# elador/FeatureDetection

Measured on AMD Instinct MI355X. Metric: Mpatches/s (extract+WVM+SVM) per GPU, 640x480 pyramid, higher is better.
Workload: dtype u8/i32/f32/f64; 1 GPU; config 1/metric config: ffpDetectApp FaceFrontal.cfg five-stage cascade on 640x480 BGR frames: 13-layer pyramid, 20x20 windows step 1 (16185 windows/frame), HistEq64 -> WVM 280 filters -> OE -> RBF-SVM 1024 SV -> NMS; fd_pyramid_update_frames + fd_detect_five_stage_frames (the frames of a call share one pyramid aren...; frames_per_call=64, calls_in_flight=11, parallelism=image-shard dp1

## Files before the change

### featuredetection_amd/capi.py

```python
import ctypes as C
import os
import numpy as np

_HERE = os.path.dirname(os.path.abspath(__file__))
LIB_PATH = os.environ.get("FD_HIP_LIB", os.path.join(_HERE, "libfd_hip.so"))

FD_OK, FD_ERR_INVALID_ARGUMENT, FD_ERR_RUNTIME, FD_ERR_LOGIC, FD_ERR_HIP, FD_ERR_CAPACITY, FD_ERR_DEVICE_CAPACITY = range(7)
FD_LAYER_NONE, FD_LAYER_GRADBIN, FD_LAYER_LBP = 0, 1, 2
IMAGE_GRAY, IMAGE_GREYWORLD_GRAY = 0, 1
FD_KERNEL_LINEAR, FD_KERNEL_POLY, FD_KERNEL_RBF, FD_KERNEL_HIK = 0, 1, 2, 3
FD_DTYPE_U8, FD_DTYPE_F32 = 0, 1


class FdError(RuntimeError):
    def __init__(self, code, msg):
        super().__init__("fd_hip error %d: %s" % (code, msg))
        self.code = code


class fd_wvm_model(C.Structure):
    _fields_ = [("filter_w", C.c_int32), ("filter_h", C.c_int32), ("num_filters", C.c_int32), ("num_used", C.c_int32),
                ("num_per_level", C.c_int32), ("basis_param", C.c_float), ("bias", C.c_float),
                ("thresholds", C.POINTER(C.c_float)), ("hk_weights", C.POINTER(C.c_float)), ("pp", C.POINTER(C.c_double)),
                ("val_off", C.POINTER(C.c_int32)), ("val", C.POINTER(C.c_double)), ("rec_off", C.POINTER(C.c_int32)),
# ... 326 lines not shown
    "fd_gradient_sum_length": (C.c_int, [C.c_int, C.c_int, C.c_int, C.c_int]),
    "fd_surf_feature_length": (C.c_int, [C.c_int, C.c_int]),
}

_BENCH_SIGS = {
    "fd_debug_svm_u8_both": (C.c_int, [C.c_void_p, C.c_void_p, C.c_void_p, C.c_int64, C.c_void_p, C.c_void_p]),
    "fd_ctx_set_kernel_timing": (C.c_int, [C.c_void_p, C.c_int]),
    "fd_last_kernel_ms": (C.c_int, [C.c_void_p, C.POINTER(C.c_char_p), C.POINTER(C.c_float)]),
    "fd_last_group_prefilter_ms": (C.c_int, [C.c_void_p, C.POINTER(C.c_float), C.POINTER(C.c_int)]),
    "fd_debug_wvb_rect_sums": (C.c_int64, [C.POINTER(fd_wvm_model), C.c_void_p, C.c_int64, C.c_void_p, C.c_void_p]),
    "fd_wvm_last_queue_length": (C.c_int64, [C.c_void_p]),
    "fd_wvm_last_tail_state": (C.c_int, [C.c_void_p]),
    "fd_wvm_last_spec_state": (C.c_int, [C.c_void_p]),
    "fd_wvm_last_stage_b_plan": (C.c_int, [C.c_void_p, C.c_void_p]),
    "fd_debug_wvd_plan": (C.c_int, [C.c_void_p, C.c_void_p, C.c_int, C.c_int, C.c_int, C.c_int, C.c_int, C.c_void_p]),
}


def lib():
    global _lib
    if _lib is None:
        if not os.path.exists(LIB_PATH):
            raise ImportError("%s not built: run `python -c 'import __graft_entry__ as g; g.build()'` "
                              "(hipcc --offload-arch=gfx950); there is no CPU fallback" % LIB_PATH)
        l = C.CDLL(LIB_PATH)
        for name, (res, args) in list(_SIGS.items()) + list(_BENCH_SIGS.items()):
            f = getattr(l, name)
            f.restype = res
            f.argtypes = args
        _lib = l
# ... 286 lines not shown

def svm_u8_both(ctx, svm, feats):
    feats = _c(feats, np.uint8).reshape(-1, svm.dim)
    o8, o16 = np.empty(len(feats), np.float64), np.empty(len(feats), np.float64)
    ctx.check(lib().fd_debug_svm_u8_both(ctx.h, svm.h, _ptr(feats), len(feats), _ptr(o8), _ptr(o16)))
    return o8, o16


def wvd_plan(nx, ny, frames, sy, ph, slots):
    nx, ny = _c(nx, np.int32), _c(ny, np.int32)
    first = np.zeros(len(nx) + 1, np.int32)
    k = lib().fd_debug_wvd_plan(_ptr(nx), _ptr(ny), len(nx), frames, sy, ph, slots, _ptr(first))
    if k < 1:
        raise FdError(k, "fd_debug_wvd_plan")
    return k, first


def wvb_rect_sums(model, patches_eq):
    s, keep = _wvm_struct(model, fd_wvm_model)
    patches_eq = _c(patches_eq, np.uint8)
    n = patches_eq.shape[0]
    gen = np.zeros(5, np.int32)
    ncols = lib().fd_debug_wvb_rect_sums(C.byref(s), None, 0, None, _ptr(gen))
    if ncols < 0:
        return None
    out = np.empty((n, ncols), np.int32)
    lib().fd_debug_wvb_rect_sums(C.byref(s), _ptr(patches_eq), n, _ptr(out), None)
    return out, [int(g) for g in gen if g >= 0]


# ... 1211 lines not shown
```

### featuredetection_amd/csrc/fd_internal.hpp

```cpp
#pragma once
#include <hip/hip_runtime.h>
#include <chrono>
#include <cstdint>
#include <cstdio>
#include <cstdlib>
#include <cmath>
#include <map>
#include <memory>
#include <string>
#include <typeindex>
#include <typeinfo>
#include <vector>
#include <stdexcept>
#include <atomic>
#include <condition_variable>
#include <functional>
#include <mutex>
#include <thread>
#include <deque>
#include <exception>
#include "../../include/fd_hip.h"
#include "../../include/fd_hip_bench.h"

struct FdPinned {
// ... 249 lines not shown
    }
    return ctx->tail;
}

static inline int fd_env_int(const char* name, int dflt, int lo, int hi) {
    const char* e = getenv(name);
    const int v = e ? atoi(e) : dflt;
    return v < lo ? lo : (v > hi ? hi : v);
}
static inline int fd_knob_batch_threads() { static const int v = fd_env_int("FD_BATCH_THREADS", 8, 1, 16); return v; }
static inline int fd_knob_wvd_rounds() { static const int v = fd_env_int("FD_WVD_ROUNDS", 2, 1, 64); return v; }
static inline bool fd_knob_trace() { static const bool on = getenv("FD_TRACE") != nullptr; return on; }
static inline int fd_knob_fs_tail() { const char* e = getenv("FD_FS_TAIL"); return e ? atoi(e) : -1; }
static inline bool fd_knob_fs_spec() { const char* e = getenv("FD_FS_SPEC"); return !(e && atoi(e) == 0); }
static inline bool fd_knob_cond_device() { const char* e = getenv("FD_COND_DEVICE"); return e && atoi(e) == 1; }

struct FdStopwatch {
    bool on = fd_knob_trace();
    std::chrono::steady_clock::time_point t;
    FdStopwatch() { restart(); }
    void restart() { if (on) t = std::chrono::steady_clock::now(); }
    int64_t lap_ns() {
        if (!on) return 0;
        const std::chrono::steady_clock::time_point n = std::chrono::steady_clock::now();
        const int64_t ns = std::chrono::duration_cast<std::chrono::nanoseconds>(n - t).count();
        t = n;
        return ns;
    }
};

// ... 127 lines not shown
```

### featuredetection_amd/csrc/pyramid.hip

```cpp
#include "fd_internal.hpp"
#include "fd_device.hpp"
#include <algorithm>
#include <cstring>

namespace {

constexpr int MAXJ = 16;

struct ResizeJob {
    int dw, dh;
    uint32_t dst_off;
    double scale_x, scale_y;
};
struct ResizeJobs {
    int n;
    ResizeJob j[MAXJ];
};
struct DownJob {
    int sw, sh;
    uint32_t src_off, dst_off;
};
struct FusedJob {
    int dw0, dh0, dw1, dh1;
    uint32_t dst0_off;
// ... 349 lines not shown
    }
#ifdef FD_PYR_PROF
    if (threadIdx.x == 0 && blockIdx.x < (unsigned int)PYR_PROF_WGS) {
        for (int i = 0; i < 6; ++i) fd_pyr_prof[blockIdx.x * 8 + i] = pacc[i];
        fd_pyr_prof[blockIdx.x * 8 + 6] = ptiles;
    }
#endif
}

__device__ __forceinline__ int reflect_cf(int p, int len) {
    int q = p < 0 ? -p : p;
    q = q >= len ? 2 * len - 2 - q : q;
    return min(max(q, 0), len - 1);
}
constexpr int PD_W = 62;
__global__ __launch_bounds__(256) void k_pyrdown_tiled(uint8_t* __restrict__ arena, DownJobs jobs, size_t imageStride) {
    __shared__ __attribute__((aligned(16))) uint8_t tile[TL_ROWS * TL_PITCH];
    arena += (size_t)blockIdx.z * imageStride;
    const int c = threadIdx.x & 63, rq = __builtin_amdgcn_readfirstlane(threadIdx.x >> 6);
    constexpr int NROWS = 2 * PD_TH + 3, PD_LD = (NROWS + 7) / 8;
    static_assert(2 * (3 + 4 * (PD_LD - 1)) + 1 < TL_ROWS && 128 <= TL_PITCH && 2 * PD_W + 3 <= 128, "pyrDown stage");
    for (int g = blockIdx.x; g < jobs.tile0[jobs.n]; g += gridDim.x) {
        int ji = 0;
        while (ji + 1 < jobs.n && g >= jobs.tile0[ji + 1]) ++ji;
        const DownJob jb = jobs.j[ji];
        const int t = g - jobs.tile0[ji];
        const int sw = jb.sw, sh = jb.sh;
        const int dw = (sw + 1) / 2, dh = (sh + 1) / 2;
        const uint8_t* src = arena + jb.src_off;
        uint8_t* dst = arena + jb.dst_off;
        const int tilesX = (dw + PD_W - 1) / PD_W;
        const int ty = t / tilesX, tx = t - ty * tilesX;
        const int dx0 = tx * PD_W, dy0 = ty * PD_TH;
        const int X0 = 2 * dx0 - 2, Y0 = 2 * dy0 - 2;
        {
            const int j4 = 4 * (c & 31), half = c >> 5;
            const int xs = X0 + j4;
// ... 633 lines not shown
        const int gx = std::max(1, std::min((int)((npix / 4 + 1023) / 1024), perFrame));
        hipLaunchKernelGGL(k_gw_stats, dim3(gx, NI), dim3(256), 0, st, fp, stats, (int)npix);
        hipLaunchKernelGGL(k_gw_gray, dim3(gx, NI), dim3(256), 0, st, fp, stats, gray, IS, (int)npix);
    } else if (frames) {
        hipLaunchKernelGGL(k_frames_to_gray, dim3(grid_for((int)(npix / 16 + 1)), NI), dim3(256), 0, st, fp, gray, IS, (int)npix, ch);
    } else if (ch == 3) {
        hipLaunchKernelGGL(k_bgr2gray, dim3(grid_for((int)npix)), dim3(256), 0, st, fp.p[0], gray, (int)npix);
    } else {
        HIP_CHECK(hipMemcpyAsync(gray, fp.p[0], npix, hipMemcpyDeviceToDevice, st));
    }
    const fd_pyramid::Plan& plan = *p->plan;
    for (const ResizeLaunch& R : plan.resize)
        hipLaunchKernelGGL(k_resize_tiled, dim3(R.grid, R.jobs.n, NI), dim3(256), 0, st, arena, arena, p->gray_full_off, W, H, R.jobs, IS);
    for (const FusedLaunch& F : plan.fused)
        hipLaunchKernelGGL(k_resize_down, dim3(F.grid), dim3(256), 0, st, arena, p->gray_full_off, W, H, p->rtab.as<int2>(), F.jobs, F.tileTab, F.tilesPerFrame, NI, IS);
    for (const DownLaunch& D : plan.down)
        hipLaunchKernelGGL(k_pyrdown_tiled, dim3(tile_grid_for(D.jobs.tile0[D.jobs.n]), 1, NI), dim3(256), 0, st, arena, D.jobs, IS);
    for (const FilterLaunch& F : plan.filter) {
        const dim3 g(F.grid, F.jobs.n);
        if (F.blur.n) hipLaunchKernelGGL(k_box_blur, g, dim3(256), 0, st, arena, p->grad_blur, F.blur);
        if (p->filter_kind != FD_LAYER_GRADBIN)
            hipLaunchKernelGGL(k_lbp, g, dim3(256), 0, st, arena, p->lbp_type, F.jobs);
        else if (p->interpolate)
            hipLaunchKernelGGL(k_gradbin<4>, g, dim3(256), 0, st, arena, p->lut.as<uint8_t>(), p->grad_kernel, F.jobs);
        else
            hipLaunchKernelGGL(k_gradbin<2>, g, dim3(256), 0, st, arena, p->lut.as<uint8_t>(), p->grad_kernel, F.jobs);
    }
    HIP_CHECK(hipGetLastError());
    if (!p->ready) HIP_CHECK(hipEventCreateWithFlags(&p->ready, hipEventDisableTiming));
    HIP_CHECK(hipEventRecord(p->ready, st));
    p->readyStream = st;
    p->version++;
// ... 383 lines not shown
```

### featuredetection_amd/csrc/wvm.hip

```cpp
#include "fd_internal.hpp"
#include "five_stage_stages.hpp"
#include <chrono>
#include <thread>
#include <algorithm>
#include <cstring>
#include <memory>
#include <mutex>
#include <atomic>


struct fd_svm;
int fd_svm_dim(const fd_svm* m);
bool fd_svm_is_u8(const fd_svm* m);
float fd_svm_threshold(const fd_svm* m);
double fd_svm_probability(const fd_svm* m, double d);
void fd_svm_generic_launch(fd_ctx* ctx, const fd_svm* m, const void* dfeat, const uint32_t* didx, int64_t stride_bytes, int64_t n, double* dout);
void fd_svm_generic_launch_on(hipStream_t st, const fd_svm* m, const void* dfeat, const uint32_t* didx, int64_t stride_bytes, int64_t n, double* dout);
bool fd_svm_u8_mfma_available(const fd_svm* m);
void fd_svm_u8_mfma_launch_counted(hipStream_t st, const fd_svm* m, const void* dfeat, const uint32_t* didx, int64_t stride_bytes, int64_t nmax,
                                   const unsigned int* dcount, double* dout);

constexpr int WVM_MAX_LAYERS = 64;
constexpr int WVM_MAX_DIM = 32;
constexpr int WVM_MAX_VALS = 16;
// ... 1146 lines not shown
        m->sbAux[i].reserve(sizeof(int2) * (size_t)cap);
        m->sbU[i].reserve(sizeof(float) * (size_t)mv.numPer * 64 * tilesCap);
        m->sbK[i].reserve(sizeof(float) * (size_t)mv.numUsed * 64 * tilesCap);
        s.X[i] = m->sbX[i].as<int8_t>(); s.wid[i] = m->sbWid[i].as<int64_t>(); s.aux[i] = m->sbAux[i].as<int2>();
        s.U[i] = m->sbU[i].as<float>(); s.K[i] = m->sbK[i].as<float>();
    }
    m->sbKey.reserve(sizeof(unsigned long long) * (size_t)cap);
    s.exitKey = m->sbKey.as<unsigned long long>();
    s.cnt = m->sbCnt.as<unsigned int>();
    s.cap = cap;
    m->deepCap = cap;
}

static int wvd_plan_sliding(WvdTable& t, int K) {
    t.K = K;
    int tiles = 0;
    for (int i = 0; i < t.n; ++i) {
        WvdLayer& l = t.l[i];
        l.G = (l.ny + K - 1) / K;
        l.sTileFirst = tiles;
        tiles += (int)(((int64_t)l.nx * l.G + 63) / 64);
    }
    t.sTilesPerImage = tiles;
    return tiles;
}
static int wvd_choose_k(WvdTable t, int slots, int ph) {
    static const int forced = [] { const char* e = getenv("FD_WVD_K"); const int v = e ? atoi(e) : 0; return v < 1 ? 0 : (v > WVD_KMAX ? WVD_KMAX : v); }();
    if (2 * t.sy > ph) return 1;
    if (forced) return forced;
    int best = 1;
    double bestCost = 0;
    for (int K = 1; K <= WVD_KMAX; ++K) {
        const int64_t tiles = (int64_t)wvd_plan_sliding(t, K) * t.nimg;
        const double rounds = (double)((tiles + slots - 1) / slots);
        const double cost = rounds * (0.45 + K * (1.0 + (K > 1 ? 0.04 * t.sy : 0.0)));
        if (K == 1 || cost < bestCost * 0.999) { best = K; bestCost = cost; }
    }
    return best;
}

template <int PW_, int PH_>
static void launch_prefilter_sized(fd_ctx* ctx, hipStream_t st, const uint8_t* arena, WvdTable wt, const WvdDev& dv) {
    static int perCu = 0;
    if (perCu == 0 && (hipOccupancyMaxActiveBlocksPerMultiprocessor(&perCu, k_wvm_prefilter<PW_, PH_>, 256, 0) != hipSuccess || perCu < 1)) perCu = 2;
    const int slots = ctx->num_cus * perCu * 4;
    const int64_t tiles = (int64_t)wvd_plan_sliding(wt, wvd_choose_k(wt, slots, PH_)) * wt.nimg;
    int grid = (int)std::min<int64_t>((tiles + 3) / 4, (int64_t)ctx->num_cus * perCu * fd_knob_wvd_rounds());
    if (wt.nimg >= 8 && grid >= 64) grid &= ~7;
    hipLaunchKernelGGL((k_wvm_prefilter<PW_, PH_>), dim3(grid), dim3(256), 0, st, arena, wt, dv);
}

static bool wvd_table_from(const WinTable& wt, WvdTable& t) {
    if (wt.raw || wt.list || wt.total < 512) return false;
    std::memset(&t, 0, sizeof(t));
    t.n = wt.n; t.sx = wt.sx; t.sy = wt.sy;
    const int64_t perImage = wt.nimg > 1 ? wt.per_image : wt.total;
    int tiles = 0;
    for (int i = 0; i < wt.n; ++i) {
        const WinLayerDev& s = wt.l[i];
        const int64_t nwin = (i + 1 < wt.n ? wt.l[i + 1].first : perImage) - s.first;
        if (nwin <= 0 || nwin > (int64_t)INT32_MAX - 64) return false;
// ... 15 lines not shown
    dv.c = m->denseC.as<WvdConst>();
    dv.q = q;
    dv.qcount = qcount;
    dv.L = m->denseL;
    dv.negBasis = m->dev.negBasis; dv.negBias = m->dev.negBias; dv.stretch = m->dev.stretch;
    dv.sxxSlack = (float)(2 * m->dev.fh + 2);
    dv.scale = m->denseScale;
    dv.nb2 = (double)m->dev.negBasis * 1.4426950408889634;
    dv.mXq = -2.0 * m->denseScale * dv.nb2;
}

static bool launch_prefilter(fd_ctx* ctx, hipStream_t st, fd_wvm* m, const uint8_t* arena, const WinTable& wt, int64_t* q, unsigned int* qcount) {
    if (m->denseL == 0) return false;
    WvdTable t;
    if (!wvd_table_from(wt, t)) return false;
    WvdDev dv;
    wvd_dev_from(m, q, qcount, dv);
#define FD_WVM_CASE(W, H) \
    if (m->dev.fw == W && m->dev.fh == H) { launch_prefilter_sized<W, H>(ctx, st, arena, t, dv); return true; }
    FD_WVM_CASE(20, 20) FD_WVM_CASE(24, 24) FD_WVM_CASE(16, 24) FD_WVM_CASE(32, 16) FD_WVM_CASE(32, 24)
#undef FD_WVM_CASE
    return false;
}

template <int PW_, int PH_>
static void launch_prefilter_group_sized(fd_ctx* ctx, hipStream_t st, const uint8_t* arena, WvdTable wt, const WvdGroup& g) {
    static int perCu = 0;
    if (perCu == 0 && (hipOccupancyMaxActiveBlocksPerMultiprocessor(&perCu, k_wvm_prefilter_group<PW_, PH_>, 256, 0) != hipSuccess || perCu < 1)) perCu = 2;
    const int slots = ctx->num_cus * perCu * 4;
    const int64_t tiles = (int64_t)wvd_plan_sliding(wt, wvd_choose_k(wt, slots, PH_)) * wt.nimg;
// ... 719 lines not shown
    std::memset(&t, 0, sizeof(t));
    t.n = n_layers; t.sx = 1; t.sy = sy; t.nimg = frames;
    for (int i = 0; i < n_layers; ++i) {
        if (nx[i] < 1 || ny[i] < 1) return FD_ERR_INVALID_ARGUMENT;
        t.l[i].nx = nx[i]; t.l[i].ny = ny[i];
    }
    const int K = wvd_choose_k(t, slots, ph);
    const int tiles = wvd_plan_sliding(t, K);
    if (tile_first) {
        for (int i = 0; i < n_layers; ++i) tile_first[i] = t.l[i].sTileFirst;
        tile_first[n_layers] = tiles;
    }
    return K;
}

int64_t fd_debug_wvb_rect_sums(const fd_wvm_model* md, const uint8_t* patches, int64_t n, int32_t* out, int32_t* phase_gen ) {
    if (!md || md->num_filters < 1) return -1;
    const int NU = (md->num_used > md->num_filters || md->num_used <= 0) ? md->num_filters : md->num_used;
    WvbTables T;
    try {
        if (!wvb_tables(md, NU, T)) return -1;
    } catch (...) { return -1; }
    const int d = md->filter_w * md->filter_h;
    int64_t ncols = 0;
    for (int k = 0; k < NU; ++k) ncols += T.lvl[4 * (size_t)k + 2] - 1;
    if (phase_gen) for (int i = 0; i <= WVB_MAXPHASE; ++i) phase_gen[i] = i <= T.nphase ? T.phaseGen[i] : -1;
    if (!out || !patches) return ncols;
    std::vector<int8_t> x((size_t)T.DS);
    for (int64_t i = 0; i < n; ++i) {
        std::fill(x.begin(), x.end(), 0);
// ... 39 lines not shown
```

### featuredetection_amd/csrc/wvm_dense.hpp

```cpp
#pragma once

constexpr int WVD_L = 16;

typedef int wvd_v4i __attribute__((ext_vector_type(4)));
typedef int wvd_v16i __attribute__((ext_vector_type(16)));
typedef __attribute__((address_space(3))) unsigned int wvd_lds_u32;
typedef __attribute__((address_space(3))) unsigned short wvd_lds_u16;

struct WvdLayer {
    int32_t bx, by, nx, lw;
    uint32_t off, magic;
    int32_t nwin, pad0;
    int64_t first;
    int32_t ny, G, sTileFirst, pad;
};
struct WvdTable {
    int32_t n, sx, sy, pad0;
    int32_t nimg, pad1;
    int32_t K, sTilesPerImage;
    int64_t perImage;
    uint64_t imageStride;
    WvdLayer l[WVM_MAX_LAYERS];
};

struct WvdScal {
    int32_t L;
    float negBasis, negBias, stretch, sxxSlack;
    int32_t pad;
    double scale, nb2, mXq;
};
struct WvdConst {
    double cA[WVD_L];
    float thr[WVD_L];
// ... 96 lines not shown
__device__ __forceinline__ void wvd_count(unsigned int ldsAddr, unsigned int inc) {
    __hip_atomic_fetch_add((wvd_lds_u32*)(uintptr_t)ldsAddr, inc, __ATOMIC_RELAXED, __HIP_MEMORY_SCOPE_WAVEFRONT);
}
__device__ __forceinline__ void wvd_uncount(unsigned int ldsAddr, unsigned int inc) {
    __hip_atomic_fetch_sub((wvd_lds_u32*)(uintptr_t)ldsAddr, inc, __ATOMIC_RELAXED, __HIP_MEMORY_SCOPE_WAVEFRONT);
}
__device__ __forceinline__ unsigned int wvd_lut(unsigned int ldsAddr) { return *(wvd_lds_u16*)(uintptr_t)ldsAddr; }
__device__ __forceinline__ unsigned int wvd_lshl_or(unsigned int a, int sh, unsigned int b) {
    unsigned int r;
    asm("v_lshl_or_b32 %0, %1, %2, %3" : "=v"(r) : "v"(a), "n"(sh), "v"(b));
    return r;
}

constexpr int WVD_KMAX = 16;

template <int NW_, bool ADD_>
__device__ __forceinline__ void wvd_hist_row(const unsigned int* w4, unsigned int blk4, unsigned int laneOff32, unsigned int inc) {
#pragma unroll
    for (int j = 0; j < NW_; ++j) {
        const unsigned int bins = wvd_bins(w4[j], blk4);
        if (ADD_) {
            wvd_count(wvd_addr<0>(bins, laneOff32), inc); wvd_count(wvd_addr<1>(bins, laneOff32), inc);
            wvd_count(wvd_addr<2>(bins, laneOff32), inc); wvd_count(wvd_addr<3>(bins, laneOff32), inc);
        } else {
            wvd_uncount(wvd_addr<0>(bins, laneOff32), inc); wvd_uncount(wvd_addr<1>(bins, laneOff32), inc);
            wvd_uncount(wvd_addr<2>(bins, laneOff32), inc); wvd_uncount(wvd_addr<3>(bins, laneOff32), inc);
        }
    }
}
__device__ __forceinline__ void wvd_swap32(unsigned int& v0, unsigned int& v1) {
// ... 40 lines not shown
            asm("" : "+v"(s1), "+v"(s2));
        }
    }
    sumx = s1;
    sumxx = s2;
}

template <int PW_, int PH_>
__global__ __launch_bounds__(256) __attribute__((amdgpu_waves_per_eu(3, 4))) void k_wvm_prefilter(const uint8_t* __restrict__ arena, WvdTable wt, WvdDev dv) {
    static_assert(PW_ % 4 == 0 && PW_ >= 16 && PW_ <= 32, "rows are read as dwords");
    constexpr int NW = PW_ / 4;
    constexpr int D4 = NW * PH_;
    static_assert(D4 % 4 == 0, "the equalise blocks take 4 dwords");
    constexpr int KS = (D4 + 7) / 8;
    __shared__ __attribute__((aligned(16384))) WvdLds S;
    const int lane = threadIdx.x & 63;
    const int wave = __builtin_amdgcn_readfirstlane(threadIdx.x >> 6);
    const __attribute__((address_space(4))) WvdConst& C = *(const __attribute__((address_space(4))) WvdConst*)(uintptr_t)dv.c;
    const int L = dv.L;
    const int K = wt.K;
    int li = 0;
    unsigned char* histPtr = reinterpret_cast<unsigned char*>(&S.hist[wave >> 1][0][wave & 1][0]);
    const unsigned int histLds = (unsigned int)(uintptr_t)(wvd_lds_u16*)histPtr;
    const unsigned int blkH4 = ((histLds >> 8) & 0xC0u) * 0x01010101u;
    const unsigned int laneOff32 = (histLds & ~0xFF00u) + (unsigned int)(lane & 31) * 4u;
    const unsigned int cntLds = histLds + (unsigned int)(lane & 31) * 4u + (unsigned int)(lane >> 5) * 2u;
    const unsigned int inc = 1u << (16 * (lane >> 5));
    const unsigned int lutLds = (unsigned int)(uintptr_t)(wvd_lds_u8*)&S.lut[0][lane][wave];
    const unsigned int blkL4 = ((lutLds >> 8) & 0xC0u) * 0x01010101u;
    const unsigned int lutWord = lutLds & ~0xFF00u;

    int lastImg = -1;
#ifdef FD_WVB_PROF
    const unsigned long long pT0 = __builtin_amdgcn_s_memtime();
    unsigned long long pAcc[4] = {0, 0, 0, 0}, pTiles = 0;
#endif
    const bool byXcd = wt.nimg >= 8 && (gridDim.x & 7u) == 0;
    const int xcd = blockIdx.x & 7, vStride = byXcd ? (int)(gridDim.x >> 3) * 4 : (int)gridDim.x * 4;
    const int vEnd = byXcd ? ((wt.nimg - xcd + 7) >> 3) * wt.sTilesPerImage : wt.sTilesPerImage * wt.nimg;
    for (int v = (byXcd ? (int)(blockIdx.x >> 3) : (int)blockIdx.x) * 4 + wave; v < vEnd; v += vStride) {
        const int fi = wt.nimg > 1 ? v / wt.sTilesPerImage : 0;
        const int img = byXcd ? xcd + 8 * fi : fi;
        const int tile = v - fi * wt.sTilesPerImage;
        if (img != lastImg) { li = 0; lastImg = img; }
        while (li + 1 < wt.n && tile >= wt.l[li + 1].sTileFirst) ++li;
        const WvdLayer& wl = wt.l[li];
        const int ntask = wl.nx * wl.G;
        const int task0 = (tile - wl.sTileFirst) * 64 + lane;
        const unsigned int task = (unsigned int)(task0 < ntask ? task0 : ntask - 1);
        unsigned int g = __umulhi(task, wl.magic);
        unsigned int ix = task - g * (unsigned int)wl.nx;
        if (ix >= (unsigned int)wl.nx) { ix -= wl.nx; ++g; }
        const int iy0 = (int)g * K;
        const int rows = task0 < ntask ? min(K, wl.ny - iy0) : 0;
        const int lw = wl.lw;
        const unsigned int rowStep = (unsigned int)(wt.sy * lw);
        const uint8_t* ubase = arena + (size_t)img * wt.imageStride + wl.off;
        const unsigned int lo0 = (unsigned int)((wl.by + iy0 * wt.sy) * lw + (wl.bx + (int)ix * wt.sx));
        const int64_t wid0 = (int64_t)img * wt.perImage + wl.first + (int64_t)iy0 * wl.nx + ix;

        WVD_T(pa);
        {
            unsigned char* z = histPtr + (lane >> 3) * 256 + (lane & 7) * 16;
#pragma unroll
            for (int i = 0; i < 8; ++i) *reinterpret_cast<uint4*>(z + i * 2048) = make_uint4(0, 0, 0, 0);
        }
        __builtin_amdgcn_wave_barrier();
        {
            unsigned int wn[NW];
#pragma unroll
            for (int j = 0; j < NW; ++j) wn[j] = wvd_load_u32(ubase + 4 * j, lo0);
#pragma unroll 2
            for (int r = 0; r < PH_; ++r) {
                unsigned int w4[NW];
#pragma unroll
                for (int j = 0; j < NW; ++j) w4[j] = wn[j];
                const uint8_t* nsrc = ubase + (size_t)(r + 1 < PH_ ? r + 1 : r) * lw;
#pragma unroll
                for (int j = 0; j < NW; ++j) wn[j] = wvd_load_u32(nsrc + 4 * j, lo0);
                wvd_hist_row<NW, true>(w4, blkH4, laneOff32, inc);
            }
        }
        WVD_T(pb0);
#ifdef FD_WVB_PROF
        pAcc[0] += pb0 - pa;
#endif
        unsigned int survBits = 0;
#pragma unroll 1
        for (int step = 0; step < K; ++step) {
        const bool active = step < rows;
        if (__ballot(active) == 0) break;
        WVD_T(ps);
        if (step > 0 && active) {
            const uint8_t* out0 = ubase + (size_t)(step - 1) * rowStep;
            for (int q = 0; q < wt.sy; ++q) {
                unsigned int wo[NW], wi[NW];
#pragma unroll
                for (int j = 0; j < NW; ++j) { wo[j] = wvd_load_u32(out0 + (size_t)q * lw + 4 * j, lo0); wi[j] = wvd_load_u32(out0 + (size_t)(q + PH_) * lw + 4 * j, lo0); }
                wvd_hist_row<NW, false>(wo, blkH4, laneOff32, inc);
                wvd_hist_row<NW, true>(wi, blkH4, laneOff32, inc);
            }
        }
        const unsigned int lo = lo0 + (unsigned int)(active ? step : (rows > 0 ? rows - 1 : 0)) * rowStep;
        wave_sync();
        WVD_T(pb);
        unsigned int sumx, sumxx;
        wvd_cdf_lut<PW_ * PH_>(cntLds, lutLds, dv.stretch, sumx, sumxx);
        wave_sync();
        WVD_T(pc);
        wvd_v16i acc00 = {}, acc01 = {}, acc10 = {}, acc11 = {};
        {
            constexpr int PF = 1;
            unsigned int nxq[PF][8];
            wvd_v4i an0, an1;
            const char* Bb = reinterpret_cast<const char*>(dv.B);
            unsigned int lane16 = (unsigned int)lane * 16u;
            asm volatile("" : "+v"(lane16));
            auto fetchPx = [&](int ks) {
#pragma unroll
                for (int j = 0; j < 8; ++j) {
                    const int q = 8 * ks + j;
                    if (q < D4) nxq[ks % PF][j] = wvd_load_u32(ubase + (size_t)(q / NW) * lw + 4 * (q % NW), lo);
                }
            };
            auto fetch = [&](int ks) {
                an0 = *reinterpret_cast<const wvd_v4i*>(Bb + (size_t)(ks * 2 + 0) * 1024 + lane16);
                an1 = *reinterpret_cast<const wvd_v4i*>(Bb + (size_t)(ks * 2 + 1) * 1024 + lane16);
            };
#pragma unroll
            for (int i = 0; i < PF; ++i)
                if (i < KS) fetchPx(i);
            fetch(0);
#pragma unroll
            for (int ks = 0; ks < KS; ++ks) {
                const wvd_v4i a0 = an0, a1 = an1;
                unsigned int cur[8], pk[8];
#pragma unroll
// ... 61 lines not shown
        {
            const unsigned long long pe = __builtin_amdgcn_s_memtime();
            pAcc[0] += pb - ps; pAcc[1] += pc - pb; pAcc[2] += pd - pc; pAcc[3] += pe - pd; ++pTiles;
        }
#endif
        }
        if (__ballot(survBits != 0)) {
            unsigned int total = 0;
            for (int st = 0; st < K; ++st) total += (unsigned int)__popcll(__ballot((survBits >> st) & 1u));
            unsigned int base = 0;
            if (lane == 0) base = atomicAdd(dv.qcount, total);
            base = __builtin_amdgcn_readfirstlane(base);
            for (int st = 0; st < K; ++st) {
                const bool mine = (survBits >> st) & 1u;
                const unsigned long long mask = __ballot(mine);
                if (mine) dv.q[base + __popcll(mask & ((1ull << lane) - 1ull))] = wid0 + (int64_t)st * wl.nx;
                base += (unsigned int)__popcll(mask);
            }
        }
        wave_sync();
    }
#ifdef FD_WVB_PROF
    if (lane == 0) {
        const unsigned int gw = blockIdx.x * 4 + wave;
        if (gw < (unsigned int)WVD_PROF_WAVES) {
            unsigned int hw, xcc;
            asm volatile("s_getreg_b32 %0, hwreg(HW_REG_HW_ID)" : "=s"(hw));
            asm volatile("s_getreg_b32 %0, hwreg(HW_REG_XCC_ID)" : "=s"(xcc));
            unsigned long long* r = fd_wvd_prof + (size_t)gw * 8;
            r[0] = pT0; r[1] = __builtin_amdgcn_s_memtime(); r[2] = (unsigned long long)hw | ((unsigned long long)xcc << 32); r[3] = pTiles;
            r[4] = pAcc[0]; r[5] = pAcc[1]; r[6] = pAcc[2]; r[7] = pAcc[3];
// ... 126 lines not shown
```

### include/fd_hip_bench.h

```cpp
#ifndef FD_HIP_BENCH_H_
#define FD_HIP_BENCH_H_
#include "fd_hip.h"
#ifdef __cplusplus
extern "C" {
#endif

int fd_ctx_set_kernel_timing(fd_ctx* ctx, int enable);
int fd_last_kernel_ms(fd_ctx* ctx, const char** kernel_name, float* ms);
int fd_last_group_prefilter_ms(fd_ctx* ctx, float* ms, int* members);

int64_t fd_wvm_last_queue_length(const fd_wvm* wvm);
int fd_wvm_last_stage_b_plan(const fd_wvm* wvm, int64_t* out);
int fd_wvm_last_tail_state(const fd_wvm* wvm);
int fd_wvm_last_spec_state(const fd_wvm* wvm);

int64_t fd_debug_wvb_rect_sums(const fd_wvm_model* md, const uint8_t* patches, int64_t n, int32_t* out, int32_t* phase_gen);

int fd_debug_wvd_plan(const int32_t* nx, const int32_t* ny, int n_layers, int frames, int sy, int ph, int slots, int32_t* tile_first);

int fd_debug_svm_u8_both(fd_ctx* ctx, const fd_svm* svm, const uint8_t* features, int64_t n, double* out8, double* out16);

#ifdef __cplusplus
}
#endif
#endif
```

Measured before the change: 3737 Mpatches/s.

## Pack WVM prefilter tasks across pyramid layers and map pyrdown frames per XCD

Adds a packed task plan for the dense WVM prefilter. Tasks from all pyramid layers are laid out contiguously, so 64-lane tiles span layer boundaries rather than leaving partial tiles at each layer's end. The K choice uses a cost model over those packed tiles. The kernel decodes each lane's layer and row group from LDS-cached layer descriptors, and address math switches to 24-bit mad with incremental row offsets. Separately, the pyrdown kernel assigns frames to blocks so that each XCD handles a fixed frame subset for cache locality. The price is per-lane layer decoding, more address-range guards, and mixed-layer tiles whose lanes have differing row counts.

```diff
diff --git a/featuredetection_amd/capi.py b/featuredetection_amd/capi.py
--- a/featuredetection_amd/capi.py
+++ b/featuredetection_amd/capi.py
@@ -364,6 +364,8 @@
     "fd_wvm_last_spec_state": (C.c_int, [C.c_void_p]),
     "fd_wvm_last_stage_b_plan": (C.c_int, [C.c_void_p, C.c_void_p]),
     "fd_debug_wvd_plan": (C.c_int, [C.c_void_p, C.c_void_p, C.c_int, C.c_int, C.c_int, C.c_int, C.c_int, C.c_void_p]),
+    "fd_debug_wvd_packed_plan": (C.c_int, [C.c_void_p, C.c_void_p, C.c_int, C.c_int, C.c_int, C.c_int, C.c_int, C.c_void_p, C.c_void_p, C.c_void_p,
+                                           C.c_int64, C.c_void_p]),
 }
 
 
@@ -680,6 +682,21 @@
     if k < 1:
         raise FdError(k, "fd_debug_wvd_plan")
     return k, first
+
+
+def wvd_packed_plan(nx, ny, frames, sy, ph, slots, tasks=None):
+    nx, ny = _c(nx, np.int32), _c(ny, np.int32)
+    tiles, ntask = C.c_int32(), C.c_int32()
+    k = lib().fd_debug_wvd_packed_plan(_ptr(nx), _ptr(ny), len(nx), frames, sy, ph, slots, C.byref(tiles), C.byref(ntask), None, 0, None)
+    if k < 1:
+        raise FdError(k, "fd_debug_wvd_packed_plan")
+    tasks = np.arange(ntask.value, dtype=np.int32) if tasks is None else _c(tasks, np.int32)
+    dec = np.zeros((len(tasks), 4), np.int32)
+    if len(tasks):
+        k = lib().fd_debug_wvd_packed_plan(_ptr(nx), _ptr(ny), len(nx), frames, sy, ph, slots, None, None, _ptr(tasks), len(tasks), _ptr(dec))
+        if k < 1:
+            raise FdError(k, "fd_debug_wvd_packed_plan")
+    return k, tiles.value, ntask.value, dec
 
 
 def wvb_rect_sums(model, patches_eq):
diff --git a/featuredetection_amd/csrc/fd_internal.hpp b/featuredetection_amd/csrc/fd_internal.hpp
--- a/featuredetection_amd/csrc/fd_internal.hpp
+++ b/featuredetection_amd/csrc/fd_internal.hpp
@@ -287,6 +287,8 @@
 static inline int fd_knob_fs_tail() { const char* e = getenv("FD_FS_TAIL"); return e ? atoi(e) : -1; }
 static inline bool fd_knob_fs_spec() { const char* e = getenv("FD_FS_SPEC"); return !(e && atoi(e) == 0); }
 static inline bool fd_knob_cond_device() { const char* e = getenv("FD_COND_DEVICE"); return e && atoi(e) == 1; }
+static inline bool fd_knob_wvd_pack() { const char* e = getenv("FD_WVD_PACK"); return !(e && atoi(e) == 0); }
+static inline bool fd_knob_pyr_xcd() { const char* e = getenv("FD_PYR_XCD"); return !(e && atoi(e) == 0); }
 
 struct FdStopwatch {
     bool on = fd_knob_trace();
diff --git a/featuredetection_amd/csrc/pyramid.hip b/featuredetection_amd/csrc/pyramid.hip
--- a/featuredetection_amd/csrc/pyramid.hip
+++ b/featuredetection_amd/csrc/pyramid.hip
@@ -387,13 +387,19 @@
     return min(max(q, 0), len - 1);
 }
 constexpr int PD_W = 62;
-__global__ __launch_bounds__(256) void k_pyrdown_tiled(uint8_t* __restrict__ arena, DownJobs jobs, size_t imageStride) {
+__global__ __launch_bounds__(256) void k_pyrdown_tiled(uint8_t* __restrict__ arena0, DownJobs jobs, size_t imageStride, int xcdFrames) {
     __shared__ __attribute__((aligned(16))) uint8_t tile[TL_ROWS * TL_PITCH];
-    arena += (size_t)blockIdx.z * imageStride;
     const int c = threadIdx.x & 63, rq = __builtin_amdgcn_readfirstlane(threadIdx.x >> 6);
     constexpr int NROWS = 2 * PD_TH + 3, PD_LD = (NROWS + 7) / 8;
     static_assert(2 * (3 + 4 * (PD_LD - 1)) + 1 < TL_ROWS && 128 <= TL_PITCH && 2 * PD_W + 3 <= 128, "pyrDown stage");
-    for (int g = blockIdx.x; g < jobs.tile0[jobs.n]; g += gridDim.x) {
+    const bool byXcd = xcdFrames > 0;
+    const int ntile = jobs.tile0[jobs.n];
+    const int first = byXcd ? (int)(blockIdx.x >> 3) : (int)blockIdx.x, stride = byXcd ? (int)(gridDim.x >> 3) : (int)gridDim.x;
+    const int items = byXcd ? (xcdFrames >> 3) * ntile : ntile;
+    for (int item = first; item < items; item += stride) {
+        const int fi = byXcd ? item / ntile : 0;
+        const int g = item - fi * ntile;
+        uint8_t* __restrict__ arena = arena0 + (size_t)(byXcd ? (int)(blockIdx.x & 7u) + 8 * fi : (int)blockIdx.z) * imageStride;
         int ji = 0;
         while (ji + 1 < jobs.n && g >= jobs.tile0[ji + 1]) ++ji;
         const DownJob jb = jobs.j[ji];
@@ -1057,8 +1063,14 @@
         hipLaunchKernelGGL(k_resize_tiled, dim3(R.grid, R.jobs.n, NI), dim3(256), 0, st, arena, arena, p->gray_full_off, W, H, R.jobs, IS);
     for (const FusedLaunch& F : plan.fused)
         hipLaunchKernelGGL(k_resize_down, dim3(F.grid), dim3(256), 0, st, arena, p->gray_full_off, W, H, p->rtab.as<int2>(), F.jobs, F.tileTab, F.tilesPerFrame, NI, IS);
-    for (const DownLaunch& D : plan.down)
-        hipLaunchKernelGGL(k_pyrdown_tiled, dim3(tile_grid_for(D.jobs.tile0[D.jobs.n]), 1, NI), dim3(256), 0, st, arena, D.jobs, IS);
+    const bool downByXcd = NI >= 8 && NI % 8 == 0 && fd_knob_pyr_xcd();
+    for (const DownLaunch& D : plan.down) {
+        const int ntile = D.jobs.tile0[D.jobs.n];
+        if (downByXcd)
+            hipLaunchKernelGGL(k_pyrdown_tiled, dim3(8 * (int)std::min<int64_t>((int64_t)(NI / 8) * ntile, 8192)), dim3(256), 0, st, arena, D.jobs, IS, NI);
+        else
+            hipLaunchKernelGGL(k_pyrdown_tiled, dim3(tile_grid_for(ntile), 1, NI), dim3(256), 0, st, arena, D.jobs, IS, 0);
+    }
     for (const FilterLaunch& F : plan.filter) {
         const dim3 g(F.grid, F.jobs.n);
         if (F.blur.n) hipLaunchKernelGGL(k_box_blur, g, dim3(256), 0, st, arena, p->grad_blur, F.blur);
diff --git a/featuredetection_amd/csrc/wvm.hip b/featuredetection_amd/csrc/wvm.hip
--- a/featuredetection_amd/csrc/wvm.hip
+++ b/featuredetection_amd/csrc/wvm.hip
@@ -1184,6 +1184,7 @@
 
 static int wvd_plan_sliding(WvdTable& t, int K) {
     t.K = K;
+    t.packed = 0;
     int tiles = 0;
     for (int i = 0; i < t.n; ++i) {
         WvdLayer& l = t.l[i];
@@ -1194,8 +1195,12 @@
     t.sTilesPerImage = tiles;
     return tiles;
 }
+static int wvd_forced_k() {
+    static const int forced = [] { const char* e = getenv("FD_WVD_K"); const int v = e ? atoi(e) : 0; return v < 1 ? 0 : (v > WVD_KMAX ? WVD_KMAX : v); }();
+    return forced;
+}
 static int wvd_choose_k(WvdTable t, int slots, int ph) {
-    static const int forced = [] { const char* e = getenv("FD_WVD_K"); const int v = e ? atoi(e) : 0; return v < 1 ? 0 : (v > WVD_KMAX ? WVD_KMAX : v); }();
+    const int forced = wvd_forced_k();
     if (2 * t.sy > ph) return 1;
     if (forced) return forced;
     int best = 1;
@@ -1209,12 +1214,74 @@
     return best;
 }
 
+static int wvd_plan_packed(WvdTable& t, int K, double* area = nullptr, double* longest = nullptr) {
+    t.K = K;
+    t.packed = 1;
+    const double step = 1.0 + (K > 1 ? 0.04 * t.sy : 0.0);
+    int64_t pos = 0, tiles = 0;
+    int cur = 0, top = 0;
+    double a = 0;
+    auto piece = [&](int rows, int64_t count) {
+        if (count <= 0) return;
+        top = std::max(top, rows);
+        if (pos & 63) {
+            const int64_t fill = std::min<int64_t>(count, 64 - (pos & 63));
+            cur = std::max(cur, rows);
+            pos += fill; count -= fill;
+            if ((pos & 63) == 0) { a += 0.45 + cur * step; ++tiles; cur = 0; }
+        }
+        const int64_t full = count >> 6;
+        a += (double)full * (0.45 + rows * step); tiles += full;
+        pos += count;
+        if (count & 63) cur = rows;
+    };
+    for (int i = 0; i < t.n; ++i) {
+        WvdLayer& l = t.l[i];
+        l.G = (l.ny + K - 1) / K;
+        l.sTileFirst = 0;
+        l.pFirst = (int32_t)pos;
+        const int q = l.ny / l.G, r = l.ny % l.G;
+        piece(q + 1, (int64_t)l.nx * r);
+        piece(q, (int64_t)l.nx * (l.G - r));
+    }
+    if (pos & 63) { a += 0.45 + cur * step; ++tiles; }
+    t.pTasks = (int32_t)pos;
+    t.sTilesPerImage = (int)tiles;
+    if (area) *area = a;
+    if (longest) *longest = 0.45 + top * step;
+    return (int)tiles;
+}
+static int wvd_choose_k_packed(WvdTable t, int slots, int ph) {
+    const int forced = wvd_forced_k();
+    if (2 * t.sy > ph) return 1;
+    if (forced) return forced;
+    int best = 1;
+    double bestCost = 0;
+    for (int K = 1; K <= WVD_KMAX; ++K) {
+        double area, longest;
+        const int perFrame = wvd_plan_packed(t, K, &area, &longest);
+        const int64_t tiles = (int64_t)perFrame * t.nimg;
+        const double cost = (double)(tiles / slots) * (area / perFrame) + (tiles % slots ? longest : 0.0);
+        if (K == 1 || cost < bestCost * 0.999) { best = K; bestCost = cost; }
+    }
+    return best;
+}
+static bool wvd_pack_ok(const WvdTable& t) {
+    int64_t tasks = 0;
+    for (int i = 0; i < t.n; ++i) tasks += t.l[i].nwin;
+    return tasks <= (int64_t)INT32_MAX - 64;
+}
+static int64_t wvd_plan(WvdTable& wt, int slots, int ph) {
+    if (fd_knob_wvd_pack() && wvd_pack_ok(wt)) return (int64_t)wvd_plan_packed(wt, wvd_choose_k_packed(wt, slots, ph)) * wt.nimg;
+    return (int64_t)wvd_plan_sliding(wt, wvd_choose_k(wt, slots, ph)) * wt.nimg;
+}
+
 template <int PW_, int PH_>
 static void launch_prefilter_sized(fd_ctx* ctx, hipStream_t st, const uint8_t* arena, WvdTable wt, const WvdDev& dv) {
     static int perCu = 0;
     if (perCu == 0 && (hipOccupancyMaxActiveBlocksPerMultiprocessor(&perCu, k_wvm_prefilter<PW_, PH_>, 256, 0) != hipSuccess || perCu < 1)) perCu = 2;
     const int slots = ctx->num_cus * perCu * 4;
-    const int64_t tiles = (int64_t)wvd_plan_sliding(wt, wvd_choose_k(wt, slots, PH_)) * wt.nimg;
+    const int64_t tiles = wvd_plan(wt, slots, PH_);
     int grid = (int)std::min<int64_t>((tiles + 3) / 4, (int64_t)ctx->num_cus * perCu * fd_knob_wvd_rounds());
     if (wt.nimg >= 8 && grid >= 64) grid &= ~7;
     hipLaunchKernelGGL((k_wvm_prefilter<PW_, PH_>), dim3(grid), dim3(256), 0, st, arena, wt, dv);
@@ -1260,6 +1327,11 @@
     if (m->denseL == 0) return false;
     WvdTable t;
     if (!wvd_table_from(wt, t)) return false;
+    for (int i = 0; i < t.n; ++i) {
+        const WvdLayer& l = t.l[i];
+        const int64_t rowsBelow = (int64_t)l.by + (int64_t)(l.ny - 1) * t.sy + m->dev.fh;
+        if ((int64_t)l.lw * std::max(t.sy, m->dev.fh) >= (1 << 24) || (int64_t)l.off + (rowsBelow + 1) * l.lw > (int64_t)UINT32_MAX) return false;
+    }
     WvdDev dv;
     wvd_dev_from(m, q, qcount, dv);
 #define FD_WVM_CASE(W, H) \
@@ -2009,6 +2081,32 @@
     return K;
 }
 
+int fd_debug_wvd_packed_plan(const int32_t* nx, const int32_t* ny, int n_layers, int frames, int sy, int ph, int slots, int32_t* tiles_per_frame,
+                             int32_t* tasks_per_frame, const int32_t* tasks, int64_t n_tasks, int32_t* decoded) {
+    if (!nx || !ny || n_layers < 1 || n_layers > WVM_MAX_LAYERS || frames < 1 || sy < 1 || ph < 1 || slots < 1 || n_tasks < 0) return FD_ERR_INVALID_ARGUMENT;
+    if (n_tasks > 0 && (!tasks || !decoded)) return FD_ERR_INVALID_ARGUMENT;
+    WvdTable t;
+    std::memset(&t, 0, sizeof(t));
+    t.n = n_layers; t.sx = 1; t.sy = sy; t.nimg = frames;
+    for (int i = 0; i < n_layers; ++i) {
+        if (nx[i] < 1 || ny[i] < 1) return FD_ERR_INVALID_ARGUMENT;
+        t.l[i].nx = nx[i]; t.l[i].ny = ny[i]; t.l[i].nwin = (int32_t)std::min<int64_t>((int64_t)nx[i] * ny[i], INT32_MAX);
+        t.l[i].magic = (uint32_t)std::min<uint64_t>((1ull << 32) / (uint64_t)nx[i], 0xffffffffull);
+    }
+    if (!wvd_pack_ok(t)) return FD_ERR_INVALID_ARGUMENT;
+    const int K = wvd_choose_k_packed(t, slots, ph);
+    const int tiles = wvd_plan_packed(t, K);
+    if (tiles_per_frame) *tiles_per_frame = tiles;
+    if (tasks_per_frame) *tasks_per_frame = t.pTasks;
+    for (int64_t i = 0; i < n_tasks; ++i) {
+        if (tasks[i] < 0 || tasks[i] >= t.pTasks) return FD_ERR_INVALID_ARGUMENT;
+        const WvdTask d = wvd_packed_task((unsigned int)tasks[i], t.n, [&](int l) { return t.l[l].pFirst; },
+                                          [&](int l) { const WvdLayer& L = t.l[l]; return make_int4(L.nx, (int)L.magic, L.ny / L.G, L.ny % L.G); });
+        decoded[4 * i] = d.li; decoded[4 * i + 1] = (int32_t)d.ix; decoded[4 * i + 2] = d.iy0; decoded[4 * i + 3] = d.rows;
+    }
+    return K;
+}
+
 int64_t fd_debug_wvb_rect_sums(const fd_wvm_model* md, const uint8_t* patches, int64_t n, int32_t* out, int32_t* phase_gen ) {
     if (!md || md->num_filters < 1) return -1;
     const int NU = (md->num_used > md->num_filters || md->num_used <= 0) ? md->num_filters : md->num_used;
diff --git a/featuredetection_amd/csrc/wvm_dense.hpp b/featuredetection_amd/csrc/wvm_dense.hpp
--- a/featuredetection_amd/csrc/wvm_dense.hpp
+++ b/featuredetection_amd/csrc/wvm_dense.hpp
@@ -10,13 +10,13 @@
 struct WvdLayer {
     int32_t bx, by, nx, lw;
     uint32_t off, magic;
-    int32_t nwin, pad0;
+    int32_t nwin, pFirst;
     int64_t first;
     int32_t ny, G, sTileFirst, pad;
 };
 struct WvdTable {
-    int32_t n, sx, sy, pad0;
-    int32_t nimg, pad1;
+    int32_t n, sx, sy, packed;
+    int32_t nimg, pTasks;
     int32_t K, sTilesPerImage;
     int64_t perImage;
     uint64_t imageStride;
@@ -143,6 +143,28 @@
 
 constexpr int WVD_KMAX = 16;
 
+__host__ __device__ __forceinline__ unsigned int wvd_mulhi(unsigned int a, unsigned int b) { return (unsigned int)(((unsigned long long)a * b) >> 32); }
+struct WvdTask { int li; unsigned int ix; int iy0, rows; };
+template <class FirstOf, class LayerOf>
+__host__ __device__ __forceinline__ WvdTask wvd_packed_task(unsigned int task, int n, FirstOf firstOf, LayerOf layerOf) {
+    WvdTask t;
+    t.li = 0;
+    unsigned int base = 0;
+    for (int l = 1; l < n; ++l) {
+        const unsigned int f = (unsigned int)firstOf(l);
+        t.li += task >= f ? 1 : 0;
+        base = task >= f ? f : base;
+    }
+    const int4 L = layerOf(t.li);
+    const unsigned int local = task - base;
+    unsigned int g = wvd_mulhi(local, (unsigned int)L.y);
+    t.ix = local - g * (unsigned int)L.x;
+    if (t.ix >= (unsigned int)L.x) { t.ix -= (unsigned int)L.x; ++g; }
+    t.iy0 = (int)g * L.z + ((int)g < L.w ? (int)g : L.w);
+    t.rows = L.z + ((int)g < L.w ? 1 : 0);
+    return t;
+}
+
 template <int NW_, bool ADD_>
 __device__ __forceinline__ void wvd_hist_row(const unsigned int* w4, unsigned int blk4, unsigned int laneOff32, unsigned int inc) {
 #pragma unroll
@@ -213,8 +235,16 @@
     static_assert(D4 % 4 == 0, "the equalise blocks take 4 dwords");
     constexpr int KS = (D4 + 7) / 8;
     __shared__ __attribute__((aligned(16384))) WvdLds S;
+    __shared__ int4 SL[WVM_MAX_LAYERS][3];
     const int lane = threadIdx.x & 63;
     const int wave = __builtin_amdgcn_readfirstlane(threadIdx.x >> 6);
+    if ((int)threadIdx.x < wt.n) {
+        const WvdLayer& l = wt.l[threadIdx.x];
+        SL[threadIdx.x][0] = make_int4(l.nx, (int)l.magic, l.ny / l.G, l.ny % l.G);
+        SL[threadIdx.x][1] = make_int4(l.lw, (int)(l.off + (unsigned int)(l.by * l.lw + l.bx)), l.ny, 0);
+        SL[threadIdx.x][2] = make_int4((int)(unsigned int)l.first, (int)(l.first >> 32), 0, 0);
+    }
+    __syncthreads();
     const __attribute__((address_space(4))) WvdConst& C = *(const __attribute__((address_space(4))) WvdConst*)(uintptr_t)dv.c;
     const int L = dv.L;
     const int K = wt.K;
@@ -241,22 +271,34 @@
         const int fi = wt.nimg > 1 ? v / wt.sTilesPerImage : 0;
         const int img = byXcd ? xcd + 8 * fi : fi;
         const int tile = v - fi * wt.sTilesPerImage;
-        if (img != lastImg) { li = 0; lastImg = img; }
-        while (li + 1 < wt.n && tile >= wt.l[li + 1].sTileFirst) ++li;
-        const WvdLayer& wl = wt.l[li];
-        const int ntask = wl.nx * wl.G;
-        const int task0 = (tile - wl.sTileFirst) * 64 + lane;
-        const unsigned int task = (unsigned int)(task0 < ntask ? task0 : ntask - 1);
-        unsigned int g = __umulhi(task, wl.magic);
-        unsigned int ix = task - g * (unsigned int)wl.nx;
-        if (ix >= (unsigned int)wl.nx) { ix -= wl.nx; ++g; }
-        const int iy0 = (int)g * K;
-        const int rows = task0 < ntask ? min(K, wl.ny - iy0) : 0;
-        const int lw = wl.lw;
-        const unsigned int rowStep = (unsigned int)(wt.sy * lw);
-        const uint8_t* ubase = arena + (size_t)img * wt.imageStride + wl.off;
-        const unsigned int lo0 = (unsigned int)((wl.by + iy0 * wt.sy) * lw + (wl.bx + (int)ix * wt.sx));
-        const int64_t wid0 = (int64_t)img * wt.perImage + wl.first + (int64_t)iy0 * wl.nx + ix;
+        int myLi, iy0, rows;
+        unsigned int ix;
+        if (wt.packed) {
+            const int task0 = tile * 64 + lane;
+            const WvdTask t = wvd_packed_task((unsigned int)min(task0, wt.pTasks - 1), wt.n, [&](int l) { return wt.l[l].pFirst; }, [&](int l) { return SL[l][0]; });
+            myLi = t.li; ix = t.ix; iy0 = t.iy0;
+            rows = task0 < wt.pTasks ? t.rows : 0;
+        } else {
+            if (img != lastImg) { li = 0; lastImg = img; }
+            while (li + 1 < wt.n && tile >= wt.l[li + 1].sTileFirst) ++li;
+            const WvdLayer& wl = wt.l[li];
+            const int ntask = wl.nx * wl.G;
+            const int task0 = (tile - wl.sTileFirst) * 64 + lane;
+            const unsigned int task = (unsigned int)(task0 < ntask ? task0 : ntask - 1);
+            unsigned int g = __umulhi(task, wl.magic);
+            ix = task - g * (unsigned int)wl.nx;
+            if (ix >= (unsigned int)wl.nx) { ix -= wl.nx; ++g; }
+            myLi = li;
+            iy0 = (int)g * K;
+            rows = task0 < ntask ? min(K, wl.ny - iy0) : 0;
+        }
+        const int4 la = SL[myLi][1], lb = SL[myLi][2];
+        const unsigned int nxl = (unsigned int)SL[myLi][0].x;
+        const unsigned int lw = (unsigned int)la.x;
+        const unsigned int rowStep = wvd_mul24((unsigned int)wt.sy, lw);
+        const uint8_t* ubase = arena + (size_t)img * wt.imageStride;
+        const unsigned int lo0 = (unsigned int)la.y + (unsigned int)(iy0 * wt.sy) * lw + ix * (unsigned int)wt.sx;
+        const int64_t wid0 = (int64_t)img * wt.perImage + (int64_t)(((unsigned long long)(unsigned int)lb.y << 32) | (unsigned int)lb.x) + (int64_t)iy0 * nxl + ix;
 
         WVD_T(pa);
         {
@@ -266,17 +308,17 @@
         }
         __builtin_amdgcn_wave_barrier();
         {
-            unsigned int wn[NW];
-#pragma unroll
-            for (int j = 0; j < NW; ++j) wn[j] = wvd_load_u32(ubase + 4 * j, lo0);
+            unsigned int wn[NW], ra = lo0;
+#pragma unroll
+            for (int j = 0; j < NW; ++j) wn[j] = wvd_load_u32(ubase + 4 * j, ra);
 #pragma unroll 2
             for (int r = 0; r < PH_; ++r) {
                 unsigned int w4[NW];
 #pragma unroll
                 for (int j = 0; j < NW; ++j) w4[j] = wn[j];
-                const uint8_t* nsrc = ubase + (size_t)(r + 1 < PH_ ? r + 1 : r) * lw;
-#pragma unroll
-                for (int j = 0; j < NW; ++j) wn[j] = wvd_load_u32(nsrc + 4 * j, lo0);
+                if (r + 1 < PH_) ra += lw;
+#pragma unroll
+                for (int j = 0; j < NW; ++j) wn[j] = wvd_load_u32(ubase + 4 * j, ra);
                 wvd_hist_row<NW, true>(w4, blkH4, laneOff32, inc);
             }
         }
@@ -291,16 +333,17 @@
         if (__ballot(active) == 0) break;
         WVD_T(ps);
         if (step > 0 && active) {
-            const uint8_t* out0 = ubase + (size_t)(step - 1) * rowStep;
-            for (int q = 0; q < wt.sy; ++q) {
+            unsigned int ro = wvd_mad24((unsigned int)(step - 1), rowStep, lo0);
+            for (int q = 0; q < wt.sy; ++q, ro += lw) {
+                const unsigned int ri = wvd_mad24((unsigned int)PH_, lw, ro);
                 unsigned int wo[NW], wi[NW];
 #pragma unroll
-                for (int j = 0; j < NW; ++j) { wo[j] = wvd_load_u32(out0 + (size_t)q * lw + 4 * j, lo0); wi[j] = wvd_load_u32(out0 + (size_t)(q + PH_) * lw + 4 * j, lo0); }
+                for (int j = 0; j < NW; ++j) { wo[j] = wvd_load_u32(ubase + 4 * j, ro); wi[j] = wvd_load_u32(ubase + 4 * j, ri); }
                 wvd_hist_row<NW, false>(wo, blkH4, laneOff32, inc);
                 wvd_hist_row<NW, true>(wi, blkH4, laneOff32, inc);
             }
         }
-        const unsigned int lo = lo0 + (unsigned int)(active ? step : (rows > 0 ? rows - 1 : 0)) * rowStep;
+        const unsigned int lo = wvd_mad24((unsigned int)(active ? step : (rows > 0 ? rows - 1 : 0)), rowStep, lo0);
         wave_sync();
         WVD_T(pb);
         unsigned int sumx, sumxx;
@@ -315,11 +358,16 @@
             const char* Bb = reinterpret_cast<const char*>(dv.B);
             unsigned int lane16 = (unsigned int)lane * 16u;
             asm volatile("" : "+v"(lane16));
+            unsigned int rowOff = lo;
+            int pr = 0;
             auto fetchPx = [&](int ks) {
 #pragma unroll
                 for (int j = 0; j < 8; ++j) {
                     const int q = 8 * ks + j;
-                    if (q < D4) nxq[ks % PF][j] = wvd_load_u32(ubase + (size_t)(q / NW) * lw + 4 * (q % NW), lo);
+                    if (q < D4) {
+                        if (pr < q / NW) { rowOff += lw; ++pr; }
+                        nxq[ks % PF][j] = wvd_load_u32(ubase + 4 * (q % NW), rowOff);
+                    }
                 }
             };
             auto fetch = [&](int ks) {
@@ -411,7 +459,7 @@
             for (int st = 0; st < K; ++st) {
                 const bool mine = (survBits >> st) & 1u;
                 const unsigned long long mask = __ballot(mine);
-                if (mine) dv.q[base + __popcll(mask & ((1ull << lane) - 1ull))] = wid0 + (int64_t)st * wl.nx;
+                if (mine) dv.q[base + __popcll(mask & ((1ull << lane) - 1ull))] = wid0 + (int64_t)((unsigned long long)(unsigned int)st * nxl);
                 base += (unsigned int)__popcll(mask);
             }
         }
diff --git a/include/fd_hip_bench.h b/include/fd_hip_bench.h
--- a/include/fd_hip_bench.h
+++ b/include/fd_hip_bench.h
@@ -18,6 +18,9 @@
 
 int fd_debug_wvd_plan(const int32_t* nx, const int32_t* ny, int n_layers, int frames, int sy, int ph, int slots, int32_t* tile_first);
 
+int fd_debug_wvd_packed_plan(const int32_t* nx, const int32_t* ny, int n_layers, int frames, int sy, int ph, int slots, int32_t* tiles_per_frame,
+                             int32_t* tasks_per_frame, const int32_t* tasks, int64_t n_tasks, int32_t* decoded);
+
 int fd_debug_svm_u8_both(fd_ctx* ctx, const fd_svm* svm, const uint8_t* features, int64_t n, double* out8, double* out16);
 
 #ifdef __cplusplus
```

Result: faster. 3863 Mpatches/s (median of 6 runs) (+3.3%).
